# SUTD-MDQS/QILaplace.jl

Hardware: AMD Instinct MI355X
Metric: MPO×MPS site-contractions/sec + max |coeff err|, n=24 χ_s=64 χ_c=128 (higher is better)
Workload: dtype f64; 1 GPU; zt_n24_chi64_D128; sites=48, mps_bonds_max=64, mpo_bonds_max=128, parallelism=replicas x1 (one signal per GPU), ranks_reported_by_collective_backend=1

## Files before the change

### qilaplace.jl_amd/csrc/qil_build_persist.hip

```cpp
#include <algorithm>
#include <cmath>
#include <cstdlib>

#include "qil_internal.h"
#include "qil_device_utils.h"

namespace {
using namespace qil_dev;

constexpr int PB_NT = 256;
constexpr int PB_NG = PB_NT / 16;
constexpr int PB_MAXL = 256;
constexpr int PB_DMAX = 56;
constexpr int PB_NCYC = 13;

struct PbArgs {
    int n, L, dcap;
    long long site_cap;
    double cutoff;
    long long maxdim;
    const double* gates;
    double* ws;
    int* dims_out;
    int* status;
    int arena_doubles;
    unsigned long long* cycles;
};

struct PbState {
    int bd[PB_MAXL + 1];
    double blk[16];
    int blk_dl, blk_dr;
    double kap[PB_DMAX], dif[PB_DMAX], beta[PB_DMAX];
    double sig[PB_DMAX], inv[PB_DMAX], nrp[PB_DMAX];
    int perm[PB_DMAX], act[PB_DMAX];
    int rank, rot, rot2, err, nact;
    double red[8];
    unsigned long long cyc[PB_NCYC], t0;
};

#define PB_FAIL(code)                      \
    do {                                   \
        if (threadIdx.x == 0) st.err = (code); \
    } while (0)

__device__ __forceinline__ void pb_tick(PbState& st, int cat, bool prof) {
    if (prof && threadIdx.x == 0) {
        const unsigned long long t = __builtin_readcyclecounter();
        st.cyc[cat] += t - st.t0;
        st.t0 = t;
    }
}

__device__ __forceinline__ void pb_put(double* W, int dl, int a, int b, double g0, double g1, double g2, double g3) {
    W[a + dl * (0 + 2 * (0 + 2 * b))] += g0;
    W[a + dl * (1 + 2 * (0 + 2 * b))] += g1;
    W[a + dl * (0 + 2 * (1 + 2 * b))] += g2;
    W[a + dl * (1 + 2 * (1 + 2 * b))] += g3;
}

__device__ void pb_main_site(int k, const double* g, int site, int* dl, int* dr, double* W) {
    const double is2 = g[0], e2is2 = g[1];
    for (int t = 0; t < 16; ++t) W[t] = 0.0;
    if (k == 1) {
        *dl = *dr = 1;
        if (site == 0) pb_put(W, 1, 0, 0, is2, is2, is2, e2is2);
        else pb_put(W, 1, 0, 0, 1, 0, 0, 1);
        return;
    }
    const int pair = site / 2 + 1;
    const bool main = (site & 1) == 0;
    if (pair < k) {
        if (main) {
            const double rf = g[2 + (k + 1 - pair)];
            *dl = pair == 1 ? 1 : 2;
            *dr = 2;
            pb_put(W, *dl, 0, 0, 1, 0, 0, 1);
            pb_put(W, *dl, pair == 1 ? 0 : 1, 1, 1, 0, 0, rf);
        } else {
            *dl = *dr = 2;
            pb_put(W, 2, 0, 0, 1, 0, 0, 1);
            pb_put(W, 2, 1, 1, 1, 0, 0, 1);
        }
        return;
    }
    if (main) {
        *dl = *dr = 2;
        pb_put(W, 2, 0, 0, is2, 0, is2, 0);
        pb_put(W, 2, 1, 1, 0, is2, 0, e2is2);
    } else {
        *dl = 2;
        *dr = 1;
        pb_put(W, 2, 0, 0, 1, 0, 0, 1);
        pb_put(W, 2, 1, 0, 1, 0, 0, 1);
    }
}

__device__ void pb_copy_site(int n, int k, const double* g, int site, int* dl, int* dr, double* W) {
    const int Lp = n - k + 1;
    for (int t = 0; t < 16; ++t) W[t] = 0.0;
    if (Lp == 1) {
        *dl = *dr = 1;
        pb_put(W, 1, 0, 0, 1, 0, 0, 1);
        return;
    }
    const int j = site / 2 + 1;
    const bool main = (site & 1) == 0;
    if (j == 1) {
        if (main) {
            *dl = 1;
            *dr = 2;
            pb_put(W, 1, 0, 0, 1, 0, 0, 1);
        } else {
            *dl = *dr = 2;
            pb_put(W, 2, 0, 0, 1, 0, 0, 0);
            pb_put(W, 2, 0, 1, 0, 0, 0, 1);
        }
        return;
    }
    if (main) {
        const double rf = g[2 + (n + 1) + (j - 2)];
        *dl = *dr = 2;
        pb_put(W, 2, 0, 0, 1, 0, 0, 1);
        pb_put(W, 2, 1, 1, 1, 0, 0, rf);
    } else {
        const bool last = j == Lp;
        *dl = 2;
        *dr = last ? 1 : 2;
        pb_put(W, 2, 0, 0, 1, 0, 0, 1);
        pb_put(W, 2, 1, last ? 0 : 1, 1, 0, 0, 1);
    }
}

__device__ void pb_block_site(PbState& st, int part, int n, int k, const double* g, int t, int nsites) {
    if (threadIdx.x != 0) return;
    int dl, dr;
    if (part == 1) {
        pb_main_site(k, g, t, &dl, &dr, st.blk);
        st.blk_dl = dl;
        st.blk_dr = dr;
    } else {
        double tmp[16];
        pb_copy_site(n, k, g, nsites - 1 - t, &dl, &dr, tmp);
        for (int a = 0; a < dl; ++a)
            for (int io = 0; io < 4; ++io)
                for (int b = 0; b < dr; ++b) st.blk[b + dr * (io + 4 * a)] = tmp[a + dl * (io + 4 * b)];
        st.blk_dl = dr;
        st.blk_dr = dl;
    }
}

template <int MU>
__device__ void pb_hh_factor_t(double* A, int lda, int m, int n, PbState& st) {
    const int tid = threadIdx.x, l16 = tid & 15, grp = tid >> 4;
    for (int j = 0; j < n; ++j) {
        double* x = A + lda * j;
        double xr[MU];
        double s2 = 0;
#pragma unroll
        for (int u = 0; u < MU; ++u) {
            const int r = l16 + 16 * u;
            xr[u] = (r > j && r < m) ? x[r] : 0.0;
        }
        const double alpha = x[j];
#pragma unroll
        for (int u = 0; u < MU; ++u) s2 = fma(xr[u], xr[u], s2);
        s2 = row16_sum(s2);
        double beta = alpha, diff = 0.0, kappa = 0.0;
        if (s2 != 0.0) {
            beta = -copysign(sqrt(fma(alpha, alpha, s2)), alpha);
            diff = alpha - beta;
            kappa = -1.0 / (beta * diff);
        }
        if (kappa != 0.0)
            for (int c0 = j + 1 + grp; c0 < n; c0 += 2 * PB_NG) {
                const int c1 = c0 + PB_NG;
                const bool two = c1 < n;
                double* y0 = A + lda * c0;
                double* y1 = A + lda * (two ? c1 : c0);
                double a0[MU], a1[MU];
#pragma unroll
                for (int u = 0; u < MU; ++u) {
                    const int r = l16 + 16 * u;
                    a0[u] = (r > j && r < m) ? y0[r] : 0.0;
                    a1[u] = (r > j && r < m) ? y1[r] : 0.0;
                }
                const double yj0 = y0[j], yj1 = y1[j];
                double w0 = 0, w1 = 0;
#pragma unroll
                for (int u = 0; u < MU; ++u) {
                    w0 = fma(xr[u], a0[u], w0);
                    w1 = fma(xr[u], a1[u], w1);
                }
                w0 = row16_sum(w0);
                w1 = row16_sum(w1);
                const double f0 = kappa * fma(diff, yj0, w0), f1 = kappa * fma(diff, yj1, w1);
#pragma unroll
                for (int u = 0; u < MU; ++u) {
                    const int r = l16 + 16 * u;
                    if (r > j && r < m) {
                        y0[r] = fma(-f0, xr[u], a0[u]);
                        if (two) y1[r] = fma(-f1, xr[u], a1[u]);
                    }
                }
                if (l16 == 0) {
                    y0[j] = fma(-f0, diff, yj0);
                    if (two) y1[j] = fma(-f1, diff, yj1);
                }
            }
        __syncthreads();
        if (tid == 0) {
            st.kap[j] = kappa;
            st.dif[j] = diff;
            st.beta[j] = beta;
            x[j] = diff;
        }
    }
    __syncthreads();
}

__device__ void pb_hh_factor(double* A, int lda, int m, int n, PbState& st) {
    if (m <= 32) pb_hh_factor_t<2>(A, lda, m, n, st);
    else if (m <= 64) pb_hh_factor_t<4>(A, lda, m, n, st);
    else if (m <= 112) pb_hh_factor_t<7>(A, lda, m, n, st);
    else pb_hh_factor_t<13>(A, lda, m, n, st);
}

__device__ void pb_hh_copy_r(const double* A, int lda, int n, const PbState& st, double* R, int ldr) {
    for (int c = threadIdx.x >> 4; c < n; c += PB_NG)
        for (int i = threadIdx.x & 15; i < n; i += 16)
            R[i + ldr * c] = i < c ? A[i + lda * c] : (i == c ? st.beta[c] : 0.0);
}

template <int MU>
__device__ void pb_hh_form_q(const double* A, int lda, int m, int n, const PbState& st, double* Q, int ldq) {
    const int tid = threadIdx.x, l16 = tid & 15, grp = tid >> 4;
    for (int pass = 0; pass * PB_NG < n; ++pass) {
        const int slot = (pass & 1) ? PB_NG - 1 - grp : grp;
        const int c = n - 1 - (pass * PB_NG + slot);
        if (c < 0) continue;
        double q[MU], xv[MU], xn[MU];
#pragma unroll
        for (int u = 0; u < MU; ++u) {
            const int r = l16 + 16 * u;
            q[u] = (r == c) ? 1.0 : 0.0;
            xv[u] = (r >= c && r < m) ? A[lda * c + r] : 0.0;
        }
        double kappa = st.kap[c];
        for (int j = c; j >= 0; --j) {
            double kn = 0.0;
            if (j > 0) {
                const double* x = A + lda * (j - 1);
                kn = st.kap[j - 1];
#pragma unroll
                for (int u = 0; u < MU; ++u) {
                    const int r = l16 + 16 * u;
                    xn[u] = (r >= j - 1 && r < m) ? x[r] : 0.0;
                }
            }
            if (kappa != 0.0) {
                double wv = 0;
#pragma unroll
                for (int u = 0; u < MU; ++u) wv = fma(xv[u], q[u], wv);
                const double f = kappa * row16_sum(wv);
#pragma unroll
                for (int u = 0; u < MU; ++u) q[u] = fma(-f, xv[u], q[u]);
            }
            kappa = kn;
#pragma unroll
            for (int u = 0; u < MU; ++u) xv[u] = xn[u];
        }
#pragma unroll
        for (int u = 0; u < MU; ++u) {
            const int r = l16 + 16 * u;
            if (r < m) Q[r + (long long)ldq * c] = q[u];
        }
    }
}

__device__ void pb_form_q(const double* A, int lda, int m, int n, const PbState& st, double* Q, int ldq) {
    if (m <= 32) pb_hh_form_q<2>(A, lda, m, n, st, Q, ldq);
    else if (m <= 64) pb_hh_form_q<4>(A, lda, m, n, st, Q, ldq);
    else if (m <= 112) pb_hh_form_q<7>(A, lda, m, n, st, Q, ldq);
    else pb_hh_form_q<13>(A, lda, m, n, st, Q, ldq);
}

__device__ void pb_gemm(const double* __restrict__ A, int lda, const double* __restrict__ Bm, int ldb,
                        double* __restrict__ C, int ldc, int m, int n, int k) {
    const int l16 = threadIdx.x & 15, grp = threadIdx.x >> 4;
    const int nrb = (m + 63) >> 6;
    int rb = 0, j = grp;
    while (j >= n && rb < nrb) {
        j -= n;
        ++rb;
    }
    while (rb < nrb) {
        const int i0 = rb * 64 + l16;
        int ro[4];
#pragma unroll
        for (int u = 0; u < 4; ++u) ro[u] = min(i0 + 16 * u, m - 1);
        const double* bj = Bm + (long long)ldb * j;
        double acc[4] = {0, 0, 0, 0};
        int kk = 0;
        for (; kk + 4 <= k; kk += 4) {
            double bv[4], av[4][4];
#pragma unroll
            for (int t = 0; t < 4; ++t) {
                bv[t] = bj[kk + t];
                const double* ak = A + (long long)lda * (kk + t);
#pragma unroll
                for (int u = 0; u < 4; ++u) av[t][u] = ak[ro[u]];
            }
#pragma unroll
            for (int t = 0; t < 4; ++t)
#pragma unroll
                for (int u = 0; u < 4; ++u) acc[u] = fma(av[t][u], bv[t], acc[u]);
        }
        if (kk < k) {
            double bv[3], av[3][4];
#pragma unroll
            for (int t = 0; t < 3; ++t) {
                const int kt = min(kk + t, k - 1);
                bv[t] = (kk + t < k) ? bj[kt] : 0.0;
                const double* ak = A + (long long)lda * kt;
#pragma unroll
                for (int u = 0; u < 4; ++u) av[t][u] = ak[ro[u]];
            }
#pragma unroll
            for (int t = 0; t < 3; ++t)
#pragma unroll
                for (int u = 0; u < 4; ++u) acc[u] = fma(av[t][u], bv[t], acc[u]);
        }
#pragma unroll
        for (int u = 0; u < 4; ++u)
            if (i0 + 16 * u < m) C[(long long)ldc * j + i0 + 16 * u] = acc[u];
        j += PB_NG;
        while (j >= n && rb < nrb) {
            j -= n;
            ++rb;
        }
    }
}

__device__ __forceinline__ void pb_copy(const double* src, double* dst, int count) {
    for (int t = threadIdx.x; t < count; t += PB_NT) dst[t] = src[t];
}

template <int G>
__device__ __forceinline__ double pb_gsum(double v) {
    v += dpp_mov<0xB1>(v);
    v += dpp_mov<0x4E>(v);
    v += dpp_mov<0x141>(v);
    if (G == 16) v += dpp_mov<0x140>(v);
    return v;
}

__device__ __forceinline__ bool pb_rotation(double al, double be, double g, double tol, double& c, double& s, bool& big) {
    const double g2 = g * g, ab = al * be;
    big = g2 > (kQuadraticOff * kQuadraticOff) * ab;
    if (!(g2 > tol * tol * ab) || g2 == 0.0) return false;
    const double d = be - al;
    const double rh = __builtin_amdgcn_rsq(fma(d, d, 4.0 * g2));
    const double c2 = fma(0.5 * fabs(d), rh, 0.5);
    const double rc = __builtin_amdgcn_rsq(c2);
    const double c0 = c2 * rc;
    const double s0 = fabs(g) * rh * rc;
    const double eps = fma(c0, c0, fma(s0, s0, -1.0));
    const double f = fma(eps, fma(eps, 0.375, -0.5), 1.0);
    c = c0 * f;
    s = copysign(s0 * f, d);
    return true;
}

template <int G, int MU>
__device__ void pb_jacobi_t(double* A, int lda, int m, int n, PbState& st, double tol, double negligible,
                            int max_sweeps, bool prof) {
    const int tid = threadIdx.x, lane = tid & (G - 1), grp = tid / G;
    constexpr int NW = PB_NT / G;
    int sweeps = 0, rounds = 0, nact = n;
    for (; sweeps < max_sweeps; ++sweeps) {
        for (int j = grp; j < n; j += NW) {
            const double* a = A + lda * j;
            double xs[MU];
#pragma unroll
            for (int u = 0; u < MU; ++u) {
                const int r = lane + G * u;
                xs[u] = r < m ? a[r] : 0.0;
            }
            double v = 0;
#pragma unroll
            for (int u = 0; u < MU; ++u) v = fma(xs[u], xs[u], v);
            v = pb_gsum<G>(v);
            if (lane == 0) st.sig[j] = v;
        }
        if (tid == 0) {
            st.rot = 0;
            st.rot2 = 0;
        }
        __syncthreads();
        if (tid < n) {
            const double mine = st.sig[tid];
            const bool keep = mine >= negligible && mine > 0.0;
            int pos = 0, tot = 0;
#pragma unroll
            for (int q = 0; q < PB_DMAX; ++q) {
                const double o = q < n ? st.sig[q] : 0.0;
                const bool kq = o >= negligible && o > 0.0;
                pos += kq && q < tid;
                tot += kq;
            }
            if (keep) {
                st.act[pos] = tid;
                st.nrp[pos] = mine;
            }
            if (tid == 0) st.nact = tot;
        }
        __syncthreads();
        nact = st.nact;
        if (nact < 2) break;
        const int npad = nact + (nact & 1);
        for (int round = 0; round < npad - 1; ++round) {
            for (int i = grp; i < npad / 2; i += NW) {
                int p, q;
                if (i == 0) {
                    p = npad - 1;
                    q = round;
                } else {
                    p = round + i;
                    q = round + npad - 1 - i;
                    if (p >= npad - 1) p -= npad - 1;
                    if (q >= npad - 1) q -= npad - 1;
                }
                if (p >= nact || q >= nact) continue;
                const int cp = st.act[p], cq = st.act[q];
                const double al = st.nrp[p], be = st.nrp[q];
                double* ap = A + lda * cp;
                double* aq = A + lda * cq;
                double x[MU], y[MU];
#pragma unroll
                for (int u = 0; u < MU; ++u) {
                    const int r = lane + G * u;
                    x[u] = r < m ? ap[r] : 0.0;
                    y[u] = r < m ? aq[r] : 0.0;
                }
                double g = 0;
#pragma unroll
                for (int u = 0; u < MU; ++u) g = fma(x[u], y[u], g);
                g = pb_gsum<G>(g);
                if (al < negligible || be < negligible) continue;
                double c, sn;
                bool big;
                if (!pb_rotation(al, be, g, tol, c, sn, big)) continue;
                if (lane == 0) {
                    st.rot = 1;
                    if (big) st.rot2 = 1;
                }
                const double sg = g >= 0 ? sn : -sn;
#pragma unroll
                for (int u = 0; u < MU; ++u) {
                    const int r = lane + G * u;
                    const double xn = fma(-sg, y[u], c * x[u]), yn = fma(sg, x[u], c * y[u]);
                    x[u] = xn;
                    y[u] = yn;
                    if (r < m) {
                        ap[r] = xn;
                        aq[r] = yn;
                    }
                }
                const double cs2 = 2.0 * c * sn * fabs(g), c2 = c * c, s2 = sn * sn;
                double aln = fma(c2, al, fma(s2, be, -cs2)), ben = fma(s2, al, fma(c2, be, cs2));
                if (aln < 0.25 * al || ben < 0.25 * be) {
                    double ea = 0, eb = 0;
#pragma unroll
                    for (int u = 0; u < MU; ++u) {
                        ea = fma(x[u], x[u], ea);
                        eb = fma(y[u], y[u], eb);
                    }
                    aln = pb_gsum<G>(ea);
                    ben = pb_gsum<G>(eb);
                }
                if (lane == 0) {
                    st.nrp[p] = aln;
                    st.nrp[q] = ben;
                }
            }
            __syncthreads();
        }
        rounds += npad - 1;
        const int any = st.rot2 ? 2 : 0;
        __syncthreads();
        if (!(any & 2)) {
            ++sweeps;
            break;
        }
    }
    for (int j = grp; j < n; j += NW) {
        const double* a = A + lda * j;
        double xs[MU];
#pragma unroll
        for (int u = 0; u < MU; ++u) {
            const int r = lane + G * u;
            xs[u] = r < m ? a[r] : 0.0;
        }
        double v = 0;
#pragma unroll
        for (int u = 0; u < MU; ++u) v = fma(xs[u], xs[u], v);
        v = pb_gsum<G>(v);
        if (lane == 0) st.sig[j] = sqrt(v);
    }
    __syncthreads();
    if (prof && tid == 0) {
        st.cyc[8] += 1;
        st.cyc[9] += n;
        st.cyc[10] += sweeps;
        st.cyc[11] += rounds;
        st.cyc[12] += nact;
    }
}

__device__ void pb_jacobi(double* A, int lda, int m, int n, PbState& st, double tol, double negligible, int max_sweeps,
                          bool prof) {
    if (n > 32) {
        if (m <= 80) pb_jacobi_t<8, 10>(A, lda, m, n, st, tol, negligible, max_sweeps, prof);
        else if (m <= 112) pb_jacobi_t<8, 14>(A, lda, m, n, st, tol, negligible, max_sweeps, prof);
        else pb_jacobi_t<8, 28>(A, lda, m, n, st, tol, negligible, max_sweeps, prof);
    } else {
        if (m <= 32) pb_jacobi_t<16, 2>(A, lda, m, n, st, tol, negligible, max_sweeps, prof);
        else if (m <= 64) pb_jacobi_t<16, 4>(A, lda, m, n, st, tol, negligible, max_sweeps, prof);
        else if (m <= 80) pb_jacobi_t<16, 5>(A, lda, m, n, st, tol, negligible, max_sweeps, prof);
        else if (m <= 112) pb_jacobi_t<16, 7>(A, lda, m, n, st, tol, negligible, max_sweeps, prof);
        else pb_jacobi_t<16, 14>(A, lda, m, n, st, tol, negligible, max_sweeps, prof);
    }
}

struct PbChain {
    double* base;
    long long cap;
    __device__ double* site(int i) const { return base + (long long)i * cap; }
};

__device__ void pb_zip(PbState& st, const PbArgs& a, PbChain ch, double* arena, int part, int k, const double* g,
                       int L2, int len, bool prof) {
    const int tid = threadIdx.x, l16 = tid & 15, grp = tid >> 4;
    const int TS = a.dcap * a.dcap;
    double* T = arena;
    double* Wk = arena + TS;
    const int WS = a.arena_doubles - TS;
    if (tid == 0) T[0] = 1.0;
    int R = 1, Da = 1, Dc = 1;
    for (int t = 0; t < L2; ++t) {
        pb_block_site(st, part, a.n, k, g, t, L2);
        const int B1 = st.bd[t + 1];
        const int E = 4 * B1;
        __syncthreads();
        const int B2 = st.blk_dr;
        const int rows = 4 * R, cols = B1 * B2;
        const int nb = rows > cols ? cols : rows;
        const bool all = Da * E + R * E * Dc + rows * cols <= WS;
        if ((!all && R * E + rows * cols > WS) || nb * cols > TS || R * Da * Dc > TS || nb > a.dcap || rows > 16 * 13) {
            PB_FAIL(1);
            __syncthreads();
            return;
        }
        const double* Ms = ch.site(t);
        double* X = Wk;
        if (all) {
            pb_copy(ch.site(t), Wk, Da * E);
            Ms = Wk;
            X = Wk + Da * E;
            __syncthreads();
        }
        double* A = X + R * E * (all ? Dc : 1);
        for (int c0 = 0; c0 < Dc; c0 += all ? Dc : 1) {
            const int c1 = all ? Dc : c0 + 1;
            for (int c = c0; c < c1; ++c) pb_gemm(T + R * Da * c, R, Ms, Da, X + R * E * (c - c0), R, R, E, Da);
            __syncthreads();
            for (int p = grp; p < 4 * cols; p += PB_NG) {
                const int i = p & 1, o = (p >> 1) & 1, col = p >> 2;
                const int b1 = col % B1, b2 = col / B1;
                for (int r0 = 0; r0 < R; r0 += 64) {
                    double acc[4];
#pragma unroll
                    for (int u = 0; u < 4; ++u) {
                        const int r = r0 + l16 + 16 * u;
                        acc[u] = (c0 > 0 && r < R) ? A[(r + R * (i + 2 * o)) + rows * col] : 0.0;
                    }
                    for (int c = c0; c < c1; ++c)
                        for (int m = 0; m < 2; ++m) {
                            const double bv = st.blk[c + Dc * (m + 2 * (o + 2 * b2))];
                            if (bv == 0.0) continue;
                            const double* xc = X + R * ((i + 2 * (m + 2 * b1)) + E * (c - c0));
#pragma unroll
                            for (int u = 0; u < 4; ++u) {
                                const int r = r0 + l16 + 16 * u;
                                if (r < R) acc[u] = fma(xc[r], bv, acc[u]);
                            }
                        }
#pragma unroll
                    for (int u = 0; u < 4; ++u) {
                        const int r = r0 + l16 + 16 * u;
                        if (r < R) A[(r + R * (i + 2 * o)) + rows * col] = acc[u];
                    }
                }
            }
            __syncthreads();
        }
        pb_tick(st, 0, prof);
        double* dst = ch.site(t);
        if (rows > cols) {
            pb_hh_factor(A, rows, rows, cols, st);
            pb_hh_copy_r(A, rows, cols, st, T, cols);
            pb_form_q(A, rows, rows, cols, st, dst, rows);
        } else {
            for (int e = tid; e < rows * rows; e += PB_NT) dst[e] = (e % rows) == (e / rows) ? 1.0 : 0.0;
            pb_copy(A, T, rows * cols);
        }
        if (tid == 0) {
            st.bd[t] = R;
            st.bd[t + 1] = nb;
        }
        __syncthreads();
        pb_tick(st, 1, prof);
        R = nb;
        Da = B1;
        Dc = B2;
    }
    if (len > L2) {
        const int dr = st.bd[L2 + 1];
        if (Da * 4 * dr > WS || R > a.dcap) {
            PB_FAIL(2);
            __syncthreads();
            return;
        }
        pb_copy(ch.site(L2), Wk, Da * 4 * dr);
        __syncthreads();
        pb_gemm(T, R, Wk, Da, ch.site(L2), R, R, 4 * dr, Da);
        if (tid == 0) st.bd[L2] = R;
    } else {
        const int dl = st.bd[L2 - 1];
        if (dl * 4 * R > WS) {
            PB_FAIL(3);
            __syncthreads();
            return;
        }
        pb_copy(ch.site(L2 - 1), Wk, dl * 4 * R);
        __syncthreads();
        pb_gemm(Wk, dl * 4, T, R, ch.site(L2 - 1), dl * 4, dl * 4, Da, R);
        if (tid == 0) st.bd[L2] = Da;
    }
    __syncthreads();
    pb_tick(st, 2, prof);
}

__device__ void pb_gauge(PbState& st, const PbArgs& a, PbChain ch, double* arena, int first, int len, bool prof) {
    const int tid = threadIdx.x;
    const int TS = a.dcap * a.dcap;
    double* Rm = arena;
    double* Wk = arena + TS;
    const int WS = a.arena_doubles - TS;
    for (int i = first; i + 1 < len; ++i) {
        const int m = st.bd[i] * 4, n = st.bd[i + 1], w2 = 4 * st.bd[i + 2];
        double* A = Wk;
        double* Nx = A + m * n;
        if (m * n + n * w2 > WS || n * n > TS || m > 16 * 13) {
            PB_FAIL(4);
            __syncthreads();
            return;
        }
        pb_copy(ch.site(i), A, m * n);
        pb_copy(ch.site(i + 1), Nx, n * w2);
        __syncthreads();
        if (m > n) {
            pb_hh_factor(A, m, m, n, st);
            pb_hh_copy_r(A, m, n, st, Rm, n);
            pb_form_q(A, m, m, n, st, ch.site(i), m);
            __syncthreads();
            pb_gemm(Rm, n, Nx, n, ch.site(i + 1), n, n, w2, n);
        } else {
            double* dst = ch.site(i);
            for (int e = tid; e < m * m; e += PB_NT) dst[e] = (e % m) == (e / m) ? 1.0 : 0.0;
            pb_gemm(A, m, Nx, n, ch.site(i + 1), m, m, w2, n);
            if (tid == 0) st.bd[i + 1] = m;
        }
        __syncthreads();
        pb_tick(st, 3, prof);
    }
}

__device__ void pb_truncate(PbState& st, const PbArgs& a, PbChain ch, double* arena, int len, bool prof) {
    const int tid = threadIdx.x, l16 = tid & 15, grp = tid >> 4, lane = tid & 63, wave = tid >> 6;
    for (int i = len - 1; i >= 1; --i) {
        const int d = st.bd[i], w = 4 * st.bd[i + 1], dl4 = 4 * st.bd[i - 1];
        const bool tall = d > w;
        const int cols = tall ? w : d, rows = tall ? d : w;
        const int ldw = rows | 1;
        double* Wk = arena;
        double* Mo = Wk + ldw * cols;
        double* VT = Mo + d * w;
        double* US = arena + a.arena_doubles - d * cols;
        double* Mp = arena;
        if (ldw * cols + d * w + (tall ? 0 : w * cols) + d * cols > a.arena_doubles ||
            dl4 * d + d * cols > a.arena_doubles || cols > PB_DMAX) {
            PB_FAIL(5);
            __syncthreads();
            return;
        }
        const double* src = ch.site(i);
        double f = 0;
        for (int t = tid; t < d * w; t += PB_NT) {
            const double v = src[t];
            Mo[t] = v;
            const int r = t % d, c = t / d;
            if (tall) Wk[r + ldw * c] = v;
            else Wk[c + ldw * r] = v;
            f = fma(v, v, f);
        }
        f = wave_sum(f);
        if (lane == 0) st.red[wave] = f;
        __syncthreads();
        f = (st.red[0] + st.red[1]) + (st.red[2] + st.red[3]);
        pb_tick(st, 4, prof);
        pb_jacobi(Wk, ldw, rows, cols, st, 1e-15, 1e-30 * f, 40, prof);
        pb_tick(st, 5, prof);
        if (tid < cols) {
            const double s = st.sig[tid];
            int pos = 0;
#pragma unroll
            for (int q = 0; q < PB_DMAX; ++q) {
                const double o = q < cols ? st.sig[q] : -1.0;
                pos += (o > s) || (o == s && q < tid);
            }
            st.perm[pos] = tid;
            st.nrp[pos] = s * s;
            st.inv[pos] = s > 0.0 ? 1.0 / s : 0.0;
        }
        __syncthreads();
        if (tid == 0) {
            int kk = cols;
            if (!(st.nrp[0] > 0.0) || cols == 1) kk = 1;
            else {
                double terr = 0.0, scale = 0.0;
                for (int q0 = 0; q0 < cols; q0 += 8) {
                    double v[8];
#pragma unroll
                    for (int u = 0; u < 8; ++u) v[u] = q0 + u < cols ? st.nrp[q0 + u] : 0.0;
#pragma unroll
                    for (int u = 0; u < 8; ++u) scale += v[u];
                }
                if (scale == 0.0) scale = 1.0;
                const double lim = a.cutoff * scale;
                bool open = true;
                for (int q0 = ((cols - 1) >> 3) << 3; q0 >= 0 && open; q0 -= 8) {
                    double v[8];
#pragma unroll
                    for (int u = 0; u < 8; ++u) v[u] = q0 + u < cols ? st.nrp[q0 + u] : 0.0;
#pragma unroll
                    for (int u = 7; u >= 0; --u) {
                        const int q = q0 + u;
                        if (q >= 1 && q < cols && open) {
                            if ((long long)(q + 1) > a.maxdim || terr + v[u] <= lim) {
                                terr += v[u];
                                kk = q;
                            } else open = false;
                        }
                    }
                }
                if (kk < 1) kk = 1;
            }
            st.rank = kk;
        }
        __syncthreads();
        const int rk = st.rank;
        double* dsti = ch.site(i);
        if (!tall) {
            for (int j = grp; j < rk; j += PB_NG) {
                const double* wj = Wk + ldw * st.perm[j];
                const double sc = st.inv[j];
                for (int c = l16; c < w; c += 16) VT[c + w * j] = wj[c] * sc;
            }
            __syncthreads();
            for (int t = tid; t < rk * w; t += PB_NT) {
                const int j = t % rk, c = t / rk;
                dsti[t] = VT[c + w * j];
            }
            pb_gemm(Mo, d, VT, w, US, d, d, rk, w);
        } else {
            for (int t = tid; t < d * rk; t += PB_NT) {
                const int r = t % d, j = t / d;
                US[t] = Wk[r + ldw * st.perm[j]];
            }
            __syncthreads();
            for (int t = tid; t < rk * w; t += PB_NT) {
                const int j = t % rk, c = t / rk;
                const double* uj = US + d * j;
                const double* mc = Mo + d * c;
                double acc = 0;
                for (int r = 0; r < d; ++r) acc = fma(uj[r], mc[r], acc);
                dsti[t] = acc * st.inv[j] * st.inv[j];
            }
        }
        __syncthreads();
        pb_copy(ch.site(i - 1), Mp, dl4 * d);
        __syncthreads();
        pb_gemm(Mp, dl4, US, d, ch.site(i - 1), dl4, dl4, rk, d);
        if (tid == 0) st.bd[i] = rk;
        __syncthreads();
        pb_tick(st, 6, prof);
    }
}

__device__ void pb_mirror(PbState& st, PbChain src, PbChain dst, int len, int* tmp_bd) {
    const int tid = threadIdx.x;
    for (int i = 0; i < len; ++i) {
        const int Da = st.bd[i], Db = st.bd[i + 1];
        const double* s = src.site(i);
        double* o = dst.site(len - 1 - i);
        for (int t = tid; t < Da * 4 * Db; t += PB_NT) {
            const int b = t % Db, io = (t / Db) & 3, aa = t / (4 * Db);
            o[t] = s[aa + Da * (io + 4 * b)];
        }
    }
    __syncthreads();
    for (int i = tid; i <= len; i += PB_NT) tmp_bd[i] = st.bd[len - i];
    __syncthreads();
    for (int i = tid; i <= len; i += PB_NT) st.bd[i] = tmp_bd[i];
    __syncthreads();
}

__global__ __launch_bounds__(PB_NT) void dt_build_persistent(PbArgs a) {
    extern __shared__ __attribute__((aligned(16))) double pb_arena[];
    __shared__ PbState st;
    __shared__ int tmp_bd[PB_MAXL + 1];
    const int tid = threadIdx.x, b = blockIdx.x;
    const bool prof = a.cycles != nullptr;
    const double* g = a.gates + (long long)b * (2 * a.n + 2);
    PbChain ch{a.ws + (long long)b * 2 * a.L * a.site_cap, a.site_cap};
    PbChain alt{ch.base + (long long)a.L * a.site_cap, a.site_cap};
    if (tid == 0) {
        st.err = 0;
        for (int c = 0; c < PB_NCYC; ++c) st.cyc[c] = 0;
        st.t0 = __builtin_readcyclecounter();
        st.bd[0] = st.bd[1] = st.bd[2] = 1;
        int dl, dr;
        pb_main_site(1, g, 0, &dl, &dr, st.blk);
        for (int t = 0; t < 4; ++t) ch.site(0)[t] = st.blk[t];
        pb_main_site(1, g, 1, &dl, &dr, st.blk);
        for (int t = 0; t < 4; ++t) ch.site(1)[t] = st.blk[t];
    }
    __syncthreads();
    int len = 2;
    for (int k = 2; k <= a.n && st.err == 0; ++k) {
        if (tid < 2) {
            double* s = ch.site(len + tid);
            s[0] = 1.0;
            s[1] = 0.0;
            s[2] = 0.0;
            s[3] = 1.0;
            st.bd[len + 1 + tid] = 1;
        }
        len += 2;
        __syncthreads();
        pb_zip(st, a, ch, pb_arena, 1, k, g, len, len, prof);
        if (st.err) break;
        pb_truncate(st, a, ch, pb_arena, len, prof);
    }
    if (a.n > 1 && st.err == 0) {
        pb_mirror(st, ch, alt, len, tmp_bd);
        for (int k = 1; k < a.n && st.err == 0; ++k) {
            const int ns = 2 * (a.n - k + 1);
            pb_zip(st, a, alt, pb_arena, 2, k, g, ns, len, prof);
            if (st.err) break;
            pb_gauge(st, a, alt, pb_arena, ns, len, prof);
            if (st.err) break;
            pb_truncate(st, a, alt, pb_arena, len, prof);
        }
        if (st.err == 0) pb_mirror(st, alt, ch, len, tmp_bd);
    }
    pb_tick(st, 7, prof);
    __syncthreads();
    for (int i = tid; i <= a.L; i += PB_NT) a.dims_out[(long long)b * (a.L + 1) + i] = st.bd[i];
    if (tid == 0) a.status[b] = st.err;
    if (prof && tid < PB_NCYC) a.cycles[(long long)b * PB_NCYC + tid] = st.cyc[tid];
}

__global__ void pb_copy_out(const double* __restrict__ ws, long long site_cap, int L, const int* __restrict__ dims,
                            double* const* __restrict__ dst) {
    const int i = blockIdx.x, b = blockIdx.y;
    const int* bd = dims + (long long)b * (L + 1);
    const int count = bd[i] * 4 * bd[i + 1];
    const double* s = ws + ((long long)b * 2 * L + i) * site_cap;
    double* o = dst[(long long)b * L + i];
    for (int t = threadIdx.x; t < count; t += blockDim.x) o[t] = s[t];
}

}

static int persist_chunk(qil_context* ctx, int64_t n, int64_t nb, const double* wrs, double cutoff, int64_t maxdim,
                         const int64_t* site_ids, qil_mpo** out, int* fallback);

int qil_build_dt_persistent(qil_context* ctx, int64_t n, int64_t nb, const double* wrs, double cutoff, int64_t maxdim,
                            const int64_t* site_ids, qil_mpo** out, int* fallback) {
    *fallback = 0;
    const int64_t per_value = 2 * (2 * n) * (52LL * 4 * 52) * (int64_t)sizeof(double);
    const int64_t chunk = std::max<int64_t>(256, (8LL << 30) / std::max<int64_t>(per_value, 1));
    for (int64_t off = 0; off < nb; off += chunk) {
        const int64_t cnt = std::min(chunk, nb - off);
        int st = persist_chunk(ctx, n, cnt, wrs + off, cutoff, maxdim, site_ids, out + off, fallback);
        if (st != QIL_OK || *fallback) {
            for (int64_t b = 0; b < off; ++b) {
                qil_mpo_destroy(out[b]);
                out[b] = nullptr;
            }
            return st;
        }
    }
    return QIL_OK;
}

static int persist_chunk(qil_context* ctx, int64_t n, int64_t nb, const double* wrs, double cutoff, int64_t maxdim,
                         const int64_t* site_ids, qil_mpo** out, int* fallback) {
    *fallback = 0;
    const int L = (int)(2 * n);
    if (L > PB_MAXL) {
        *fallback = 1;
        return QIL_OK;
    }
    const int B = (int)nb;
    int dcap = 52;
    if (const char* e = getenv("QIL_DT_DCAP")) dcap = std::max(8, std::min(PB_DMAX, atoi(e)));
    const long long site_cap = (long long)dcap * 4 * dcap;
    const int arena_doubles = (160 * 1024 - 8 * 1024) / 8;
    static qil_lds_grant grant;
    if (grant.ensure(ctx->device, reinterpret_cast<const void*>(&dt_build_persistent), (size_t)arena_doubles * 8) != hipSuccess) {
        (void)hipGetLastError();
        *fallback = 1;
        return QIL_OK;
    }
    const int gstride = 2 * (int)n + 2;
    std::vector<double> gates((size_t)B * gstride, 0.0);
    for (int b = 0; b < B; ++b) {
        double* g = gates.data() + (size_t)b * gstride;
        const double w = wrs[b], is2 = 1.0 / std::sqrt(2.0);
        g[0] = is2;
        g[1] = std::exp(-w / 2.0) * is2;
        for (int idx = 0; idx <= n; ++idx) g[2 + idx] = std::exp(-w * std::pow(2.0, -idx));
        for (int e = 0; e + 1 < n; ++e) g[2 + (n + 1) + e] = std::exp(-w * std::pow(2.0, e));
    }
    void *dg = nullptr, *ws = nullptr, *dmeta = nullptr, *dcyc = nullptr;
    const size_t meta_ints = (size_t)B * (L + 1) + (size_t)B;
    QIL_TRY(qil_ctx_alloc(ctx, gates.size() * sizeof(double), &dg));
    QIL_TRY(qil_ctx_alloc(ctx, (size_t)B * 2 * L * site_cap * sizeof(double), &ws));
    QIL_TRY(qil_ctx_alloc(ctx, meta_ints * sizeof(int), &dmeta));
    const bool prof = getenv("QIL_DT_PROFILE") != nullptr;
    if (prof) {
        QIL_TRY(qil_ctx_alloc(ctx, (size_t)B * PB_NCYC * sizeof(unsigned long long), &dcyc));
    }
    QIL_HIP(hipMemcpyAsync(dg, gates.data(), gates.size() * sizeof(double), hipMemcpyHostToDevice, qil_stream(ctx)));
    PbArgs a;
    a.n = (int)n;
    a.L = L;
    a.dcap = dcap;
    a.site_cap = site_cap;
    a.cutoff = std::max(cutoff, 1e-28);
    a.maxdim = maxdim <= 0 ? INT64_MAX : maxdim;
    a.gates = static_cast<const double*>(dg);
    a.ws = static_cast<double*>(ws);
    a.dims_out = static_cast<int*>(dmeta);
    a.status = a.dims_out + (size_t)B * (L + 1);
    a.arena_doubles = arena_doubles;
    a.cycles = static_cast<unsigned long long*>(dcyc);
    if (prof) QIL_TRY(qil_timer_start(ctx));
    hipLaunchKernelGGL(dt_build_persistent, dim3(B), dim3(PB_NT), (size_t)arena_doubles * 8, qil_stream(ctx), a);
    QIL_HIP(hipGetLastError());
    double kernel_ms = 0.0;
    if (prof) QIL_TRY(qil_timer_stop(ctx, &kernel_ms));
    std::vector<int> meta(meta_ints);
    QIL_HIP(hipMemcpyAsync(meta.data(), dmeta, meta_ints * sizeof(int), hipMemcpyDeviceToHost, qil_stream(ctx)));
    QIL_HIP(qil_stream_sync(ctx));
    if (prof) {
        std::vector<unsigned long long> cyc((size_t)B * PB_NCYC);
        QIL_HIP(hipMemcpy(cyc.data(), dcyc, cyc.size() * sizeof(unsigned long long), hipMemcpyDeviceToHost));
        static const char* names[8] = {"zip-core", "zip-qr", "zip-absorb", "gauge-qr", "svd-load", "svd-jacobi",
                                             "svd-post", "other"};
        unsigned long long tot = 0;
        for (int c = 0; c < 8; ++c) tot += cyc[c];
        int nfail = 0;
        for (int b = 0; b < B; ++b) nfail += meta[(size_t)B * (L + 1) + b] != 0;
        fprintf(stderr, "[qil dt persistent] kernel %.3f ms, %d of %d values over capacity (code of value 0: %d); value 0, "
                "n=%lld: %.3f Mcycles:", kernel_ms, nfail, B, meta[(size_t)B * (L + 1)], (long long)n, tot * 1e-6);
        for (int c = 0; c < 8; ++c) fprintf(stderr, " %s %.1f%%", names[c], 100.0 * cyc[c] / std::max<double>(tot, 1));
        const double ns = std::max<double>((double)cyc[8], 1.0);
        fprintf(stderr, "; %llu SVDs, mean columns %.1f, sweeps %.2f, rounds %.1f, columns left in the last sweep %.1f\n",
                cyc[8], cyc[9] / ns, cyc[10] / ns, cyc[11] / ns, cyc[12] / ns);
        unsigned long long tmin = ~0ull, tmax = 0;
        int bmax = 0;
        double tsum = 0;
        for (int b = 0; b < B; ++b) {
            unsigned long long tb = 0;
            for (int c = 0; c < 8; ++c) tb += cyc[(size_t)b * PB_NCYC + c];
            tsum += (double)tb;
            if (tb < tmin) tmin = tb;
            if (tb > tmax) {
                tmax = tb;
                bmax = b;
            }
        }
        fprintf(stderr, "[qil dt persistent] cycles per value: min %.1f M, mean %.1f M, max %.1f M (value %d, wr = %.3f); kernel time x 2.4 GHz = %.1f M; slowest value:",
                tmin * 1e-6, tsum / B * 1e-6, tmax * 1e-6, bmax, wrs[bmax], kernel_ms * 2.4);
        {
            const unsigned long long* cb = cyc.data() + (size_t)bmax * PB_NCYC;
            for (int c = 0; c < 8; ++c) fprintf(stderr, " %s %.1f%%", names[c], 100.0 * cb[c] / std::max<double>((double)tmax, 1));
            const double nsb = std::max<double>((double)cb[8], 1.0);
            fprintf(stderr, "; %llu SVDs, mean columns %.1f, sweeps %.2f, rounds %.1f (%.0f cycles per round)\n", cb[8], cb[9] / nsb, cb[10] / nsb, cb[11] / nsb,
                    (double)cb[5] / std::max<double>((double)cb[11], 1.0));
        }
        qil_ctx_free(ctx, dcyc);
    }
    const int* status = meta.data() + (size_t)B * (L + 1);
    bool over = false;
    for (int b = 0; b < B; ++b) over = over || status[b] != 0;
    if (over) {
        qil_ctx_free(ctx, dg);
        qil_ctx_free(ctx, ws);
        qil_ctx_free(ctx, dmeta);
        *fallback = 1;
        return QIL_OK;
    }
    std::vector<double*> ptrs((size_t)B * L);
    std::vector<int64_t> bonds((size_t)std::max(L - 1, 1));
    int st = QIL_OK;
    int made = 0;
    for (int b = 0; b < B && st == QIL_OK; ++b) {
        const int* bd = meta.data() + (size_t)b * (L + 1);
        for (int i = 0; i + 1 < L; ++i) bonds[(size_t)i] = bd[i + 1];
        qil_mpo* W = nullptr;
        st = qil_mpo_alloc(ctx, L, QIL_F64, 1, bonds.data(), site_ids, &W);
        if (st != QIL_OK) break;
        out[b] = W;
        ++made;
        for (int i = 0; i < L; ++i) ptrs[(size_t)b * L + i] = static_cast<double*>(W->site[(size_t)i]);
    }
    void* dptr = nullptr;
    if (st == QIL_OK) st = qil_ctx_alloc(ctx, ptrs.size() * sizeof(double*), &dptr);
    if (st == QIL_OK) {
        hipError_t e = hipMemcpyAsync(dptr, ptrs.data(), ptrs.size() * sizeof(double*), hipMemcpyHostToDevice, qil_stream(ctx));
        if (e == hipSuccess) {
            hipLaunchKernelGGL(pb_copy_out, dim3(L, B), dim3(256), 0, qil_stream(ctx), (const double*)ws, site_cap, L,
                               (const int*)dmeta, (double* const*)dptr);
            e = hipGetLastError();
        }
        if (e == hipSuccess) e = qil_stream_sync(ctx);
        if (e != hipSuccess) st = qil_fail(QIL_EHIP, "build_dt_mpo: copy-out failed: %s", hipGetErrorString(e));
    }
    if (dptr) qil_ctx_free(ctx, dptr);
    qil_ctx_free(ctx, dg);
    qil_ctx_free(ctx, ws);
    qil_ctx_free(ctx, dmeta);
    if (st != QIL_OK) {
        for (int b = 0; b < made; ++b) {
            qil_mpo_destroy(out[b]);
            out[b] = nullptr;
        }
    }
    return st;
}
```

Before: 3842 site-contractions/s.

## Run small one-sided Jacobi SVDs on a single wavefront with wave-level fences

```diff
diff --git a/qilaplace.jl_amd/csrc/qil_build_persist.hip b/qilaplace.jl_amd/csrc/qil_build_persist.hip
--- a/qilaplace.jl_amd/csrc/qil_build_persist.hip
+++ b/qilaplace.jl_amd/csrc/qil_build_persist.hip
@@ -51,6 +51,12 @@
         st.t0 = t;
     }
 }
+
+typedef __attribute__((address_space(3))) double pb_lds_t;
+typedef __attribute__((address_space(1))) double pb_glb_t;
+__device__ __forceinline__ pb_lds_t* pb_lds(double* p) { return (pb_lds_t*)p; }
+__device__ __forceinline__ const pb_lds_t* pb_lds(const double* p) { return (const pb_lds_t*)p; }
+__device__ __forceinline__ pb_glb_t* pb_glb(double* p) { return (pb_glb_t*)p; }
 
 __device__ __forceinline__ void pb_put(double* W, int dl, int a, int b, double g0, double g1, double g2, double g3) {
     W[a + dl * (0 + 2 * (0 + 2 * b))] += g0;
@@ -151,10 +157,11 @@
 }
 
 template <int MU>
-__device__ void pb_hh_factor_t(double* A, int lda, int m, int n, PbState& st) {
+__device__ void pb_hh_factor_t(double* Ag, int lda, int m, int n, PbState& st) {
     const int tid = threadIdx.x, l16 = tid & 15, grp = tid >> 4;
+    pb_lds_t* A = pb_lds(Ag);
     for (int j = 0; j < n; ++j) {
-        double* x = A + lda * j;
+        pb_lds_t* x = A + lda * j;
         double xr[MU];
         double s2 = 0;
 #pragma unroll
@@ -176,8 +183,8 @@
             for (int c0 = j + 1 + grp; c0 < n; c0 += 2 * PB_NG) {
                 const int c1 = c0 + PB_NG;
                 const bool two = c1 < n;
-                double* y0 = A + lda * c0;
-                double* y1 = A + lda * (two ? c1 : c0);
+                pb_lds_t* y0 = A + lda * c0;
+                pb_lds_t* y1 = A + lda * (two ? c1 : c0);
                 double a0[MU], a1[MU];
 #pragma unroll
                 for (int u = 0; u < MU; ++u) {
@@ -226,15 +233,19 @@
     else pb_hh_factor_t<13>(A, lda, m, n, st);
 }
 
-__device__ void pb_hh_copy_r(const double* A, int lda, int n, const PbState& st, double* R, int ldr) {
+__device__ void pb_hh_copy_r(const double* Ag, int lda, int n, const PbState& st, double* Rg, int ldr) {
+    const pb_lds_t* A = pb_lds(Ag);
+    pb_lds_t* R = pb_lds(Rg);
     for (int c = threadIdx.x >> 4; c < n; c += PB_NG)
         for (int i = threadIdx.x & 15; i < n; i += 16)
             R[i + ldr * c] = i < c ? A[i + lda * c] : (i == c ? st.beta[c] : 0.0);
 }
 
 template <int MU>
-__device__ void pb_hh_form_q(const double* A, int lda, int m, int n, const PbState& st, double* Q, int ldq) {
+__device__ void pb_hh_form_q(const double* Ag, int lda, int m, int n, const PbState& st, double* Qg, int ldq) {
     const int tid = threadIdx.x, l16 = tid & 15, grp = tid >> 4;
+    const pb_lds_t* A = pb_lds(Ag);
+    pb_glb_t* Q = pb_glb(Qg);
     for (int pass = 0; pass * PB_NG < n; ++pass) {
         const int slot = (pass & 1) ? PB_NG - 1 - grp : grp;
         const int c = n - 1 - (pass * PB_NG + slot);
@@ -250,7 +261,7 @@
         for (int j = c; j >= 0; --j) {
             double kn = 0.0;
             if (j > 0) {
-                const double* x = A + lda * (j - 1);
+                const pb_lds_t* x = A + lda * (j - 1);
                 kn = st.kap[j - 1];
 #pragma unroll
                 for (int u = 0; u < MU; ++u) {
@@ -372,11 +383,177 @@
     return true;
 }
 
+__device__ __forceinline__ void pb_wave_fence() {
+    __builtin_amdgcn_fence(__ATOMIC_RELEASE, "wavefront");
+    __builtin_amdgcn_wave_barrier();
+    asm volatile("" ::: "memory");
+    __builtin_amdgcn_fence(__ATOMIC_ACQUIRE, "wavefront");
+}
+
+__device__ __forceinline__ void pb_pair(int npad, int round, int i, int& p, int& q) {
+    if (i == 0) {
+        p = npad - 1;
+        q = round;
+    } else {
+        p = round + i;
+        q = round + npad - 1 - i;
+        if (p >= npad - 1) p -= npad - 1;
+        if (q >= npad - 1) q -= npad - 1;
+    }
+}
+
+template <int MU>
+__device__ __forceinline__ void pb_norms_wave0(const double* A, int lda, int m, int n, int lane, int grp, double& v0, double& v1) {
+    const double* a0 = A + lda * (grp < n ? grp : 0);
+    const double* a1 = A + lda * (grp + 8 < n ? grp + 8 : 0);
+    double xs[MU], ys[MU];
+#pragma unroll
+    for (int u = 0; u < MU; ++u) {
+        const int r = lane + 8 * u;
+        xs[u] = r < m ? a0[r] : 0.0;
+        ys[u] = r < m ? a1[r] : 0.0;
+    }
+    v0 = 0;
+    v1 = 0;
+#pragma unroll
+    for (int u = 0; u < MU; ++u) {
+        v0 = fma(xs[u], xs[u], v0);
+        v1 = fma(ys[u], ys[u], v1);
+    }
+    v0 = pb_gsum<8>(v0);
+    v1 = pb_gsum<8>(v1);
+}
+
+template <int MU>
+__device__ __forceinline__ bool pb_rounds_wave0(double* A, int lda, int m, int nact, PbState& st, double tol, double negligible) {
+    const int tid = threadIdx.x, lane = tid & 7, i = tid >> 3;
+    const int npad = nact + (nact & 1);
+    int p, q;
+    pb_pair(npad, 0, i, p, q);
+    bool valid = i < npad / 2 && p < nact && q < nact;
+    int cp = valid ? st.act[p] : 0, cq = valid ? st.act[q] : 0;
+    bool bigs = false;
+    for (int round = 0; round < npad - 1; ++round) {
+        double* ap = A + lda * cp;
+        double* aq = A + lda * cq;
+        double x[MU], y[MU];
+#pragma unroll
+        for (int u = 0; u < MU; ++u) {
+            const int r = lane + 8 * u;
+            x[u] = (valid && r < m) ? ap[r] : 0.0;
+            y[u] = (valid && r < m) ? aq[r] : 0.0;
+        }
+        const double al = valid ? st.nrp[p] : 0.0, be = valid ? st.nrp[q] : 0.0;
+        int pn, qn;
+        pb_pair(npad, round + 1, i, pn, qn);
+        const bool validn = round + 2 < npad && i < npad / 2 && pn < nact && qn < nact;
+        const int cpn = validn ? st.act[pn] : 0, cqn = validn ? st.act[qn] : 0;
+        double g0 = 0, g1 = 0;
+#pragma unroll
+        for (int u = 0; u < MU; ++u) {
+            if (u & 1) g1 = fma(x[u], y[u], g1);
+            else g0 = fma(x[u], y[u], g0);
+        }
+        const double g = pb_gsum<8>(g0 + g1);
+        double c, sn;
+        bool big = false;
+        if (valid && !(al < negligible || be < negligible) && pb_rotation(al, be, g, tol, c, sn, big)) {
+            bigs = bigs || big;
+            const double sg = g >= 0 ? sn : -sn;
+#pragma unroll
+            for (int u = 0; u < MU; ++u) {
+                const int r = lane + 8 * u;
+                const double xn = fma(-sg, y[u], c * x[u]), yn = fma(sg, x[u], c * y[u]);
+                x[u] = xn;
+                y[u] = yn;
+                if (r < m) {
+                    ap[r] = xn;
+                    aq[r] = yn;
+                }
+            }
+            const double cs2 = 2.0 * c * sn * fabs(g), c2 = c * c, s2 = sn * sn;
+            double aln = fma(c2, al, fma(s2, be, -cs2)), ben = fma(s2, al, fma(c2, be, cs2));
+            if (aln < 0.25 * al || ben < 0.25 * be) {
+                double ea = 0, eb = 0;
+#pragma unroll
+                for (int u = 0; u < MU; ++u) {
+                    ea = fma(x[u], x[u], ea);
+                    eb = fma(y[u], y[u], eb);
+                }
+                aln = pb_gsum<8>(ea);
+                ben = pb_gsum<8>(eb);
+            }
+            if (lane == 0) {
+                st.nrp[p] = aln;
+                st.nrp[q] = ben;
+            }
+        }
+        pb_wave_fence();
+        p = pn;
+        q = qn;
+        cp = cpn;
+        cq = cqn;
+        valid = validn;
+    }
+    return __ballot(bigs) != 0;
+}
+
+template <int MU>
+__device__ __forceinline__ void pb_jacobi_wave0(double* A, int lda, int m, int n, PbState& st, double tol, double negligible,
+                                                int max_sweeps, bool prof) {
+    const int tid = threadIdx.x, lane = tid & 7, grp = tid >> 3;
+    int sweeps = 0, rounds = 0, nact = n;
+    double v0, v1;
+    for (; sweeps < max_sweeps; ++sweeps) {
+        pb_norms_wave0<MU>(A, lda, m, n, lane, grp, v0, v1);
+        if (lane == 0) {
+            if (grp < n) st.sig[grp] = v0;
+            if (grp + 8 < n) st.sig[grp + 8] = v1;
+        }
+        pb_wave_fence();
+        const double mine = tid < n ? st.sig[tid] : 0.0;
+        const bool keep = tid < n && mine >= negligible && mine > 0.0;
+        const unsigned long long kept = __ballot(keep);
+        if (keep) {
+            const int pos = __popcll(kept & ((1ull << tid) - 1ull));
+            st.act[pos] = tid;
+            st.nrp[pos] = mine;
+        }
+        nact = __popcll(kept);
+        pb_wave_fence();
+        if (nact < 2) break;
+        const bool big = pb_rounds_wave0<MU>(A, lda, m, nact, st, tol, negligible);
+        rounds += nact + (nact & 1) - 1;
+        if (!big) {
+            ++sweeps;
+            break;
+        }
+    }
+    pb_norms_wave0<MU>(A, lda, m, n, lane, grp, v0, v1);
+    if (lane == 0) {
+        if (grp < n) st.sig[grp] = sqrt(v0);
+        if (grp + 8 < n) st.sig[grp + 8] = sqrt(v1);
+    }
+    if (prof && tid == 0) {
+        st.cyc[8] += 1;
+        st.cyc[9] += n;
+        st.cyc[10] += sweeps;
+        st.cyc[11] += rounds;
+        st.cyc[12] += nact;
+    }
+}
+
 template <int G, int MU>
 __device__ void pb_jacobi_t(double* A, int lda, int m, int n, PbState& st, double tol, double negligible,
                             int max_sweeps, bool prof) {
     const int tid = threadIdx.x, lane = tid & (G - 1), grp = tid / G;
     constexpr int NW = PB_NT / G;
+    constexpr int MU8 = G == 16 ? 2 * MU : MU;
+    if (n <= 16) {
+        if (tid < 64) pb_jacobi_wave0<MU8>(A, lda, m, n, st, tol, negligible, max_sweeps, prof);
+        __syncthreads();
+        return;
+    }
     int sweeps = 0, rounds = 0, nact = n;
     for (; sweeps < max_sweeps; ++sweeps) {
         for (int j = grp; j < n; j += NW) {
@@ -419,6 +596,13 @@
         nact = st.nact;
         if (nact < 2) break;
         const int npad = nact + (nact & 1);
+        if (nact <= 16) {
+            if (tid < 64) {
+                const bool big = pb_rounds_wave0<MU8>(A, lda, m, nact, st, tol, negligible);
+                if (tid == 0 && big) st.rot2 = 1;
+            }
+            __syncthreads();
+        } else
         for (int round = 0; round < npad - 1; ++round) {
             for (int i = grp; i < npad / 2; i += NW) {
                 int p, q;
```

Result: slower. 3638 site-contractions/s (-5.3%).
